# VISION-SJTU/UniDefense

Measured on AMD Instinct MI355X. Metric: images/sec fwd+bwd (256x256, EffNet-b4), higher is better.
Workload: dtype f32

## Files before the change

include/unidefense_hip.h:

```cpp
#ifndef UNIDEFENSE_HIP_H
#define UNIDEFENSE_HIP_H
#include <stdint.h>

#ifdef __cplusplus
extern "C" {
#endif

#define UD_EINVAL (-1000)

typedef void* ud_stream_t;

typedef struct {
    int N, Hin, Win, Cin, Hout, Wout, KH, KW, stride, pad_t, pad_l, transposed;
} ud_conv_geom;

typedef struct {
    const float* A; const float* B; float* C;
    int M, N, K;
    long lda, ldb, ldc;
    int a_mode, b_mode, out_mode, split_k;
    int batch; long strideA, strideB, strideC;
    ud_conv_geom g;
    double* stat_sum; double* stat_sumsq;
    int half_mask;
// ... 139 lines not shown
int ud_avgpool_fwd(const float* x, float* y, int N, int Ho, int Wo, int C, int k, ud_stream_t stream);
int ud_avgpool_bwd(const float* dy, float* dx, int N, int Ho, int Wo, int C, int k, ud_stream_t stream);
int ud_adaptive_avgpool_fwd(const float* x, float* y, int N, int H, int W, int Ho, int Wo, int C, ud_stream_t stream);
int ud_adaptive_avgpool_bwd(const float* dy, float* dx, int N, int H, int W, int Ho, int Wo, int C, ud_stream_t stream);
int ud_maxpool3s2_fwd(const float* x, float* y, unsigned char* arg, int N, int H, int W, int C,
                      ud_stream_t stream);
int ud_maxpool3s2_bwd(const float* dy, const unsigned char* arg, float* dx, int N, int H, int W, int C,
                      ud_stream_t stream);
int ud_add_act_fwd(const float* a, const float* b, int act, float* y, long total, ud_stream_t stream);
int ud_relu_bwd(const float* dy, const float* y, float* g, long total, ud_stream_t stream);
int ud_copy_cols(float* narrow, float* wide, long M, int Cn, int Cw, int off, int dir, ud_stream_t stream);

int ud_aw_triplet(const float* feat, int N, int D, int n_real, float* loss, float* dfeat, float* ws,
                  ud_stream_t stream);

typedef struct {
    const float* feat[3]; float* dfeat[3]; int D[3]; int nfeat;
    const float* cls; const long long* tgt; float* dcls; int N, C, R, F;
    const float* fm; float* dfm; int nfm; const float* sm; float* dsm; int nsm;
    const float* spatial; float* dspatial; const float* freq; float* dfreq;
    float w_cls, w_fm, w_sm, w_trip, w_rec, w_freq;
    float* vals;
    float* ws;
} ud_loss_tail;
int ud_loss_tail_ws_floats(int N, int n_real, int nfeat);
int ud_loss_tail_run(const ud_loss_tail* t, ud_stream_t stream);

int ud_conv_small_supported(int Cin, int Cout, int KH, int KW);
int ud_conv_small(const ud_conv_geom* g, const float* x, const float* wmat, float* y, int Cout, ud_stream_t stream);
int ud_conv_small_wgrad_supported(int Cin, int Ma, int KH, int KW);
long ud_conv_small_wgrad_ws_floats(int Cin, int Ma);
int ud_conv_small_wgrad(const ud_conv_geom* g, const float* a, const float* x, float* part, float* out, int Ma,
                        ud_stream_t stream);

int ud_stem_dgrad_supported(int Cin, int Cout, int KH, int KW, int stride);
int ud_stem_dgrad(const ud_conv_geom* g, const float* dy, const float* w, float* dx, int Cout, int accumulate,
                  ud_stream_t stream);
int ud_absdiff_bwd(const float* a, const float* b, const float* g, float* da, float* db, long total, ud_stream_t stream);
int ud_outer(const float* u, const float* v, float* out, long M, int D, ud_stream_t stream);

int ud_attack_step_linf(float* x_adv, const float* x0, const float* g, long total, float step, float eps, float lo, float hi,
                        ud_stream_t stream);
long ud_sample_sumsq_ws_bytes(int N, long per);
int ud_sample_sumsq(const float* a, const float* b, int N, long per, double* out, double* ws, long ws_bytes,
                    ud_stream_t stream);
int ud_attack_step_l2(float* x_adv, const float* g, const double* gss, int N, long per, float step, ud_stream_t stream);
int ud_attack_project_l2(float* x_adv, const float* x0, const double* dss, int N, long per, float eps, float lo, float hi,
                         ud_stream_t stream);

#define UD_APGD_MAX_CHECKPOINTS 16
#define UD_APGD_I_K 0
#define UD_APGD_I_CNT 1
#define UD_APGD_I_HALVED 2
#define UD_APGD_I_IMPROVED 3
#define UD_APGD_I_RESET 4
#define UD_APGD_F_PREV 0
#define UD_APGD_F_BEST 1
#define UD_APGD_F_CKPT 2
#define UD_APGD_F_ETA 3
#define UD_APGD_F_A 4
int ud_apgd_control(const float* f, int* ist, float* fst, float* history, int N, int steps, const int* ck_w,
                    const int* ck_thr, int n_ck, float eta0, float alpha, int closing, ud_stream_t stream);
int ud_apgd_update_linf(float* x, float* x_prev, float* x_best, float* g_best, const float* x0, const float* g, const int* ist,
                        const float* fst, int N, long per, float eps, float lo, float hi, ud_stream_t stream);
int ud_apgd_keep(float* dst, const float* src, const int* flag, int N, long per, ud_stream_t stream);
int ud_apgd_step_l2(float* x, float* z, float* x_best, float* g_best, double* gss_best, const float* g, const double* gss,
// ... 231 lines not shown
```

unidefense_amd/attack.py:

```python
import contextlib
import inspect
import math

import torch
import torch.nn.functional as F

from .infer import _MAX_RUNNERS, _check_model, _check_precision, _eval_nodes

DEFAULT_GRAD_SCALE = 1024.0

NORMS = ("linf", "l2")
OBJECTIVES = ("cross_entropy",)


def cross_entropy_sum(out, y):
    cls = out["cls_out"]
    if cls.shape[1] == 1:
        return F.binary_cross_entropy_with_logits(cls.squeeze(1), y.to(cls.dtype), reduction="sum")
    return F.cross_entropy(cls, y, reduction="sum")


def _objective(objective):
    if callable(objective):
        return objective
    if objective not in OBJECTIVES:
        raise ValueError(f"objective must be one of {OBJECTIVES} or a callable (out, y) -> scalar, got {objective!r}")
    return cross_entropy_sum


@contextlib.contextmanager
def frozen(model):
    flags = [(p, p.requires_grad) for p in model.parameters()]
    try:
# ... 63 lines not shown
    return objective if isinstance(objective, str) else getattr(objective, "__name__", repr(objective))


class _Runner:
    _what = "runner"
    _backward = True

    def _init_model(self, model, batch, size, precision, arguments):
        self.precision, self.half = precision, precision == "fp16"
        self.device = _check_model(self._what, model, precision, arguments)
        self.model, self.batch, self.size = model, int(batch), int(size)
        self.shape = (self.batch, 3, self.size, self.size)
        self.calls = 0
        self.graph = self.out = None

    def _init_loss(self, objective, grad_scale):
        self.grad_scale = resolve_grad_scale(self.precision, grad_scale)
        self.objective = _objective(objective)
        self.g = None

    def _check(self, x, y):
        if not isinstance(x, torch.Tensor) or not x.is_cuda or not isinstance(y, torch.Tensor) or not y.is_cuda:
            raise ValueError(f"{self._what} takes cuda tensors")
        if tuple(x.shape) != self.shape or x.dtype != torch.float32:
            raise ValueError(f"input {tuple(x.shape)} {x.dtype} differs from the runner's key {self.shape} torch.float32")
        if tuple(y.shape) != (self.batch,) or y.dtype != torch.int64:
            raise ValueError(f"labels {tuple(y.shape)} {y.dtype} differ from the runner's key ({self.batch},) torch.int64")
        if self.model.training:
            raise ValueError("the model is in training mode: call model.eval() before the runner")

    def _capture(self, *bodies):
        torch.cuda.synchronize(self.device)
        graphs = [torch.cuda.CUDAGraph() for _ in bodies]
        with frozen(self.model) if self._backward else contextlib.nullcontext():
            for g, body in zip(graphs, bodies):
                with torch.cuda.graph(g):
                    body()
        return graphs

    def _nodes(self):
        return _eval_nodes(self.model, half=True) if self.half else contextlib.nullcontext()

    def _grad(self, x, value):
        from . import kernels as K
        with self._nodes():
            out = self.model(x)
            f = value(out)
            total = f if f.dim() == 0 else f.sum()
            g, = torch.autograd.grad(total * self.grad_scale if self.half else total, x)
        if self.half:
            g = g.contiguous()
            K.axpby(g, 1.0 / self.grad_scale, out=g)
        return g, _detached(out), f

    def _each(self, out):
        f = self.objective(out, self.y)
        if not isinstance(f, torch.Tensor) or tuple(f.shape) != (self.batch,):
            raise ValueError(f"{self._what}'s objective must return a [{self.batch}] tensor, one value per sample, got "
                             f"{tuple(f.shape) if isinstance(f, torch.Tensor) else type(f).__name__}")
        return f

    def _draw(self, sample, generator):
        gdev = generator.device if generator is not None else self.device
        return sample(self.shape, generator=generator, device=gdev, dtype=torch.float32).to(self.device)

    def _box_start(self, x, generator):
        return (x + (self._draw(torch.rand, generator) * 2.0 - 1.0) * self.eps).clamp_(self.lo, self.hi)

    def _merge(self, restart, better):
        from . import kernels as K
# ... 635 lines not shown
```

unidefense_amd/kernels.py:

```python
import ctypes as C
import math
import os

import torch

from . import lib as _lib
from .config import cfg as CFG
from .devmem import Scratch, ZeroPool
from .lib import ConvGeom, GemmDesc, GemmP3Desc

_call = _lib.call

GEMM_PROFILE = None


def _stream():
    return C.c_void_p(torch.cuda.current_stream().cuda_stream)


def _p(t):
    if t is None:
        return None
    return C.c_void_p(t.data_ptr())

# ... 1046 lines not shown
def conv_geom(N, Hin, Win, Cin, Hout, Wout, KH, KW, stride, pad_t, pad_l, transposed=0):
    g = ConvGeom()
    g.N, g.Hin, g.Win, g.Cin, g.Hout, g.Wout = N, Hin, Win, Cin, Hout, Wout
    g.KH, g.KW, g.stride, g.pad_t, g.pad_l, g.transposed = KH, KW, stride, pad_t, pad_l, transposed
    return g


_CONV_SPLITK = True


_CONV_SMALL = True
_CONV_SMALL_MIN_M = 262144
_CONV_SMALL_OK = {}


def _conv_small_supported(Ci, Co, KH, KW):
    key = (Ci, Co, KH, KW)
    if key not in _CONV_SMALL_OK:
        _CONV_SMALL_OK[key] = _call("ud_conv_small_supported", Ci, Co, KH, KW) == 1
    return _CONV_SMALL_OK[key]


_CONV_SMALL_WS = Scratch(torch.float32)
_CONV_SMALL_WGRAD_OK = {}


def _conv_small_wgrad_supported(Ci, Ma, KH, KW):
    key = (Ci, Ma, KH, KW)
    if key not in _CONV_SMALL_WGRAD_OK:
        _CONV_SMALL_WGRAD_OK[key] = _call("ud_conv_small_wgrad_supported", Ci, Ma, KH, KW) == 1
    return _CONV_SMALL_WGRAD_OK[key]


def conv_gather_nt(x, wmat, g):
    _chk(x, wmat)
    M = g.N * g.Hout * g.Wout
    K = g.KH * g.KW * g.Cin
    Co = wmat.shape[0]
    assert wmat.shape[1] == K and x.numel() == g.N * g.Hin * g.Win * g.Cin
    if _CONV_SMALL and M >= _CONV_SMALL_MIN_M and _conv_small_supported(g.Cin, Co, g.KH, g.KW):
        out = empty((g.N, g.Hout, g.Wout, Co), x)
        _call("ud_conv_small", C.byref(g), _p(x), _p(wmat), _p(out), Co, _stream())
        return out
    split = _fwd_split(M, Co, K) if _CONV_SPLITK else 1
    if g.Cin % 4 == 0:
        gk = (g.Hin, g.Win, g.Cin, g.KH, g.KW, g.stride, g.transposed)
        tmp = []

        def scratch():
            if not tmp:
                tmp.append(empty((M, Co), x))
            return tmp[0]
        tuned = _tuned_plan(("conv",) + gk, M, Co, K,
                            lambda cfg, sp: _gemm(x, wmat, scratch(), M, Co, K, 0, K, Co, 2, 0, 2 if sp > 1 else 0, sp, geom=g, cfg=cfg),
                            lambda: _gemm(x, wmat, scratch(), M, Co, K, 0, K, Co, 2, 0, 2 if split > 1 else 0, split, geom=g))
        if tuned is not None:
            cfg, sp = tuned
            out = (split_out if sp > 1 else empty)((g.N, g.Hout, g.Wout, Co), x)
            _gemm(x, wmat, out, M, Co, K, 0, K, Co, 2, 0, 2 if sp > 1 else 0, sp, geom=g, cfg=cfg)
            return out
    if split > 1:
        out = split_out((g.N, g.Hout, g.Wout, Co), x)
        _gemm(x, wmat, out, M, Co, K, 0, K, Co, 2, 0, 2, split, geom=g)
        return out
    out = empty((g.N, g.Hout, g.Wout, Co), x)
    _gemm(x, wmat, out, M, Co, K, 0, K, Co, 2, 0, geom=g)
    return out


_STEM_DGRAD_OK = {}


# ... 266 lines not shown
def square_propose(x_try, x_best, x0, ist, side, dh, dw, dsign, eps, lo, hi, closing=False):
    _chk_same(x_try, x_best, x0)
    if x_try.dim() != 4 or x_try.shape[1] != 3 or x_try.shape[2] != x_try.shape[3]:
        raise ValueError(f"expected [N, 3, size, size] images, got {tuple(x_try.shape)}")
    N, size, steps = x_try.shape[0], x_try.shape[2], side.numel()
    _chk_state(ist, None, N, SQUARE_I, SQUARE_F)
    _chk_i32(side, (steps,), "side")
    _chk_i32(dh, (steps, N), "dh")
    _chk_i32(dw, (steps, N), "dw")
    _chk(dsign)
    if tuple(dsign.shape) != (steps, N, 3):
        raise ValueError(f"dsign must be [{steps}, {N}, 3], got {tuple(dsign.shape)}")
    _call("ud_square_propose", _p(x_try), _p(x_best), _p(x0), _p(ist), _p(side), _p(dh), _p(dw), _p(dsign), N, size, steps,
          float(eps), float(lo), float(hi), int(bool(closing)), _stream())
    return x_try


def square_control(f, ist, fst, history, decisions, steps, early_stop=True):
    _chk(f, history)
    N = f.numel()
    _chk_state(ist, fst, N, SQUARE_I, SQUARE_F)
    if tuple(history.shape) != (int(steps) + 1, N):
        raise ValueError(f"history must be [{int(steps) + 1}, {N}], got {tuple(history.shape)}")
    _chk_i32(decisions, (int(steps) + 1, N), "decisions")
    _call("ud_square_control", _p(f), _p(ist), _p(fst), _p(history), _p(decisions), N, int(steps), int(bool(early_stop)), _stream())


def conv_gather_wgrad(a, x, g):
    _chk(a, x)
    Kdim = g.N * g.Hout * g.Wout
    Ma = a.shape[-1]
    assert a.numel() == Kdim * Ma
    Ncols = g.KH * g.KW * g.Cin
    if _CONV_SMALL and Kdim >= _CONV_SMALL_MIN_M and _conv_small_wgrad_supported(g.Cin, Ma, g.KH, g.KW):
        ws = _CONV_SMALL_WS.get(a, _call("ud_conv_small_wgrad_ws_floats", g.Cin, Ma))
        out = empty((Ma, Ncols), a)
        _call("ud_conv_small_wgrad", C.byref(g), _p(a), _p(x), _p(ws), _p(out), Ma, _stream())
        return out
    split = _pick_split(_tiles(Ma, Ncols), Kdim)
    if g.Cin % 4 == 0 and Ma % 4 == 0:
        gk = (g.Hin, g.Win, g.Cin, g.KH, g.KW, g.stride, g.transposed)
        tmp = []

        def scratch():
            if not tmp:
                tmp.append(empty((Ma, Ncols), a))
            return tmp[0]
        tuned = _tuned_plan(("convw",) + gk, Ma, Ncols, Kdim,
                            lambda cfg, sp: _gemm(a, x, scratch(), Ma, Ncols, Kdim, Ma, 0, Ncols, 1, 2, 2 if sp > 1 else 0, sp, geom=g, cfg=cfg),
                            lambda: _gemm(a, x, scratch(), Ma, Ncols, Kdim, Ma, 0, Ncols, 1, 2, 2 if split > 1 else 0, split, geom=g))
        if tuned is not None:
            cfg, sp = tuned
            out = (split_out if sp > 1 else empty)((Ma, Ncols), a)
            return _gemm(a, x, out, Ma, Ncols, Kdim, Ma, 0, Ncols, 1, 2, 2 if sp > 1 else 0, sp, geom=g, cfg=cfg)
    if split > 1:
        out = split_out((Ma, Ncols), a)
        return _gemm(a, x, out, Ma, Ncols, Kdim, Ma, 0, Ncols, 1, 2, 2, split, geom=g)
    out = empty((Ma, Ncols), a)
    return _gemm(a, x, out, Ma, Ncols, Kdim, Ma, 0, Ncols, 1, 2, 0, 1, geom=g)


_REDUCE_WS = Scratch(torch.float64, 1 << 20)


def _ws64(ref, need):
    return _p(_REDUCE_WS.get(ref, need)) if need > 0 else None
# ... 1481 lines not shown
```

unidefense_amd/lib.py:

```python
import ctypes as C
import os

_HERE = os.path.dirname(os.path.abspath(__file__))
from .config import cfg as _cfg

LIB_PATH = _cfg.lib_path or os.path.join(_HERE, "libunidefense_hip.so")


class UDLibraryError(RuntimeError):
    pass


class ConvGeom(C.Structure):
    _fields_ = [(n, C.c_int) for n in ("N", "Hin", "Win", "Cin", "Hout", "Wout", "KH", "KW", "stride",
                                       "pad_t", "pad_l", "transposed")]


class GemmDesc(C.Structure):
    _fields_ = [("A", C.c_void_p), ("B", C.c_void_p), ("C", C.c_void_p),
                ("M", C.c_int), ("N", C.c_int), ("K", C.c_int),
                ("lda", C.c_long), ("ldb", C.c_long), ("ldc", C.c_long),
                ("a_mode", C.c_int), ("b_mode", C.c_int), ("out_mode", C.c_int), ("split_k", C.c_int),
                ("batch", C.c_int), ("strideA", C.c_long), ("strideB", C.c_long), ("strideC", C.c_long),
                ("g", ConvGeom), ("stat_sum", C.c_void_p), ("stat_sumsq", C.c_void_p), ("half_mask", C.c_int), ("tile_cfg", C.c_int), ("slice_stride", C.c_long)]
# ... 92 lines not shown
    "ud_gate_mix_fwd": [_P, _P, _P, _P, _L, _P],
    "ud_gate_mix_bwd": [_P, _P, _P, _P, _P, _P, _P, _P, _L, _P],
    "ud_residual_fwd": [_P, _P, _P, _F, _P, _L, _L, _P],
    "ud_axpby": [_P, _F, _P, _F, _P, _L, _I, _P],
    "ud_mask_scale": [_P, _P, _F, _P, _L, _P],
    "ud_absdiff": [_P, _P, _P, _L, _P],
    "ud_bcast_rows": [_P, _F, _P, _I, _I, _I, _P],
    "ud_pix_to_planes": [_P, _P, _I, _I, _I, _I, _P],
    "ud_planes_to_pix": [_P, _P, _P, _I, _I, _I, _I, _P],
    "ud_bilinear_fwd": [_P, _P, _I, _I, _I, _I, _I, _P],
    "ud_bilinear_bwd": [_P, _P, _I, _I, _I, _I, _I, _P],
    "ud_l1_chunks": [_L],
    "ud_l1_fwd": [_P, _P, _P, _P, _I, _L, _F, _P],
    "ud_l1_bwd": [_P, _P, _P, _F, _I, _P, _I, _L, _P],
    "ud_dynfilter_fwd": [_P, _P, _P, _P, _P, _P, _P, _P, _I, _I, _I, _I, _P],
    "ud_dynfilter_bwd": [_P, _P, _P, _P, _P, _P, _P, _P, _P, _I, _I, _I, _P],
    "ud_avgpool_fwd": [_P, _P, _I, _I, _I, _I, _I, _P],
    "ud_avgpool_bwd": [_P, _P, _I, _I, _I, _I, _I, _P],
    "ud_adaptive_avgpool_fwd": [_P, _P, _I, _I, _I, _I, _I, _I, _P],
    "ud_adaptive_avgpool_bwd": [_P, _P, _I, _I, _I, _I, _I, _I, _P],
    "ud_maxpool3s2_fwd": [_P, _P, _P, _I, _I, _I, _I, _P],
    "ud_maxpool3s2_bwd": [_P, _P, _P, _I, _I, _I, _I, _P],
    "ud_add_act_fwd": [_P, _P, _I, _P, _L, _P],
    "ud_relu_bwd": [_P, _P, _P, _L, _P],
    "ud_copy_cols": [_P, _P, _L, _I, _I, _I, _I, _P],
    "ud_aw_triplet": [_P, _I, _I, _I, _P, _P, _P, _P],
    "ud_loss_tail_ws_floats": [_I, _I, _I],
    "ud_loss_tail_run": [C.POINTER(LossTail), _P],
    "ud_conv_small_supported": [_I, _I, _I, _I],
    "ud_conv_small": [C.POINTER(ConvGeom), _P, _P, _P, _I, _P],
    "ud_conv_small_wgrad_supported": [_I, _I, _I, _I],
    "ud_conv_small_wgrad_ws_floats": [_I, _I],
    "ud_conv_small_wgrad": [C.POINTER(ConvGeom), _P, _P, _P, _P, _I, _P],
    "ud_stem_dgrad_supported": [_I, _I, _I, _I, _I],
    "ud_stem_dgrad": [C.POINTER(ConvGeom), _P, _P, _P, _I, _I, _P],
    "ud_attack_step_linf": [_P, _P, _P, _L, _F, _F, _F, _F, _P],
    "ud_sample_sumsq_ws_bytes": [_I, _L],
    "ud_sample_sumsq": [_P, _P, _I, _L, _P, _P, _L, _P],
    "ud_attack_step_l2": [_P, _P, _P, _I, _L, _F, _P],
    "ud_attack_project_l2": [_P, _P, _P, _I, _L, _F, _F, _F, _P],
    "ud_apgd_control": [_P, _P, _P, _P, _I, _I, C.POINTER(C.c_int), C.POINTER(C.c_int), _I, _F, _F, _I, _P],
    "ud_apgd_update_linf": [_P, _P, _P, _P, _P, _P, _P, _P, _I, _L, _F, _F, _F, _P],
    "ud_apgd_keep": [_P, _P, _P, _I, _L, _P],
    "ud_apgd_step_l2": [_P, _P, _P, _P, _P, _P, _P, _P, _P, _I, _L, _P],
    "ud_apgd_combine_l2": [_P, _P, _P, _P, _I, _L, _P],
    "ud_apgd_project_l2": [_P, _P, _P, _P, _I, _L, _F, _F, _F, _P],
    "ud_fmn_norms_ws_bytes": [_I, _L],
    "ud_fmn_norm_parts": [_P, _P, _P, _I, _L, _P, _L, _P],
    "ud_fmn_control": [_P, _P, _L, _P, _P, _P, _P, _P, _P, _P, _P, _I, _L, _I, _I, _I, _P],
    "ud_fmn_update": [_P, _P, _P, _P, _P, _P, _P, _I, _L, _I, _F, _F, _P],
    "ud_fmn_project_l2": [_P, _P, _P, _P, _I, _L, _F, _F, _P],
    "ud_square_propose": [_P, _P, _P, _P, _P, _P, _P, _P, _I, _I, _I, _F, _F, _F, _I, _P],
    "ud_square_control": [_P, _P, _P, _P, _P, _I, _I, _I, _P],
    "ud_absdiff_bwd": [_P, _P, _P, _P, _P, _L, _P],
    "ud_outer": [_P, _P, _P, _L, _I, _P],
    "ud_gather2d": [_P, _P, _P, _P, _L, _I, _I, _P],
    "ud_blur5_reflect": [_P, _P, _L, _I, _I, _F, _F, _F, _P],
    "ud_amp_mix": [_P, _P, _P, _P, _L, _I, _I, _I, _P],
    "ud_efdm_ws_bytes": [_I, _I],
    "ud_efdm": [_P, _P, _P, _P, _I, _I, _I, _P, _L, _P],
    "ud_coral_moments": [_P, _P, _I, _I, _I, _P],
    "ud_affine3": [_P, _P, _P, _I, _I, _P],
    "ud_fused_reduce_ws_doubles": [_I, _I, _I, _I, _I],
    "ud_colstats": [_P, _I, _I, _I, _P, _P, _P, _I, _P],
    "ud_colsum_bn": [_P, _BN, _I, _I, _I, _P, _P, _I, _P],
    "ud_coldot_bn": [_P, _P, _BN, _I, _I, _I, _P, _P, _I, _P],
# ... 41 lines not shown
    "ud_rfft2_ex": [_P, _P, _I, _I, _I, _F, _F, _BN, _P, _P, _I, _P, _P, _I, _P, _P],
    "ud_rfft2_ex_planes": [_P, _P, _L, _L, _P, _F, _P, _I, _I, _I, _F, _F, _BN, _P, _P, _I, _P, _P, _P, _P, _I, _P],
    "ud_irfft2_mix": [_P, _P, _I, _I, _I, _F, _F, _P, _P, _P, _P, _P, _I, _P],
    "ud_rfft2_two_pass": [_P, _P, _P, _I, _I, _I, _F, _F, _BN, _P, _P, _I, _P, _P, _I, _P, _P],
    "ud_irfft2_two_pass": [_P, _P, _P, _I, _I, _I, _F, _F, _P, _P, _P, _P, _P, _I, _P],
    "ud_fft2_two_pass_ws_floats": [_I, _I, _I],
    "ud_dwtile_ws_doubles": [_I, _I, _I, _I],
    "ud_dwtile": [_P, _BN, _P, _P] + [_I] * 10 + [_P, _I, _P, _P, _BN, _I, _P, _P, _P, _I, _I, _P],
    "ud_dwtile_wgrad_part_rows": [_I, _I, _I],
    "ud_dwtile_wgrad": [_P, _BN, _P, _P, _I, _P, _P, _L] + [_I] * 9 + [_I, _I, _P],
    "ud_dwtile_wgrad_finalize": [_P, _I, _I, _I, _P, _I, _P, _P],
    "ud_dwtile_wgrad_finalize_multi": [C.POINTER(WgradFold), _I, _P],
    "ud_rfft2_ex_plane_half": [_P, _P, _L, _P, _I, _I, _I, _F, _F, _BN, _P, _P, _I, _P, _P, _P, _P, _I, _P],
    "ud_irfft2_dwbwd": [_P, _I, _I, _I, _F, _F, _P, _P, _BN, _P, _I, _P, _I, _P, _P, _P, _P, _P, _I, _P],
    "ud_dwtile_dgrad_eval": [_P, _P, _P, _I, _P, _P, _BN, _P] + [_I] * 11 + [_P],
    "ud_dwtile_bwd": [_P, _P, _BN, _P, _P, _I, _P, _P, _P, _P, _L, _P, _P, _P] + [_I] * 8 + [_P],
    "ud_rfft2_planes_ws_floats": [_L, _I],
    "ud_rfft2_planes": [_P, _P, _P, _L, _I, _F, _P],
    "ud_rfft2_planes_adjoint": [_P, _P, _P, _L, _I, _F, _P],
    "ud_adamw_chunk_elems": [],
    "ud_adamw_multi": [_P, _P, _I, _P, _P, _I, C.c_double, C.c_double, C.c_double, _I, _I, _P, _P, _P, _P, _P],
    "ud_multi_add": [_P, _P, _P, _I, _P],
    "ud_gemm_get_path": [],
    "ud_sum_slices": [_P, _P, _I, _L, _L, _I, _P],
    "ud_xchg_bytes": [_I, _I, _I],
    "ud_xchg_create": [_I, _I, _I, _P, _P],
    "ud_xchg_open": [_P, _P],
    "ud_xchg_close": [_P],
    "ud_xchg_destroy": [_P],
    "ud_xchg_allreduce": [_P, _I, _P, _I, _I, _I, _I, _P, _P, _L, _P, _P],
}

_COUNT_FUNCS = {"ud_mb_eval_dw_ok", "ud_mb_eval_dw_tiles", "ud_mb_eval_dw_h_ok", "ud_mb_eval_dw_h_tiles", "ud_pj_fwd_fused_ok", "ud_pj_bwd_fused_ok", "ud_pj_bwd_fused_grid", "ud_pw_bwd_fused_ok", "ud_pw_bwd_fused_grid", "ud_loss_tail_ws_floats", "ud_dwtile_wgrad", "ud_dwtile_bwd", "ud_fft32_set_wave", "ud_fft2_two_pass_ws_floats", "ud_dwtile_ws_doubles", "ud_dwtile_wgrad_part_rows", "ud_reduce_ws_doubles", "ud_gemm_query_path", "ud_gemm_get_path", "ud_gemm_stats_slots", "ud_adamw_chunk_elems", "ud_rfft2_planes_ws_floats", "ud_fused_reduce_ws_doubles", "ud_dwconv_bwd_data_bn_ws_doubles", "ud_dwconv_bwd_weight_parts", "ud_sfmix_blocks", "ud_gate_mix_blocks",
                "ud_l1_chunks", "ud_efdm_ws_bytes", "ud_conv_small_supported", "ud_conv_small_wgrad_supported",
                "ud_conv_small_wgrad_ws_floats", "ud_xchg_bytes", "ud_stem_dgrad_supported", "ud_sample_sumsq_ws_bytes",
                "ud_coldot_bn_eval_ws_doubles", "ud_fmn_norms_ws_bytes"}
_LONG_FUNCS = {"ud_mb_eval_dw_tiles", "ud_mb_eval_dw_h_tiles", "ud_pj_bwd_fused_grid", "ud_pw_bwd_fused_grid", "ud_fft2_two_pass_ws_floats", "ud_dwtile_ws_doubles", "ud_dwtile_wgrad_part_rows", "ud_xchg_bytes", "ud_efdm_ws_bytes", "ud_rfft2_planes_ws_floats", "ud_conv_small_wgrad_ws_floats", "ud_fused_reduce_ws_doubles",
               "ud_dwconv_bwd_data_bn_ws_doubles", "ud_sample_sumsq_ws_bytes", "ud_coldot_bn_eval_ws_doubles",
               "ud_fmn_norms_ws_bytes"}

EXPORTED = tuple(_SIGNATURES)

_lib = None


def load():
    global _lib
    if _lib is not None:
        return _lib
    if not os.path.exists(LIB_PATH):
        raise UDLibraryError(
            f"{LIB_PATH} is missing: build it with `python -c 'import __graft_entry__ as g; g.build()'` "
            "or `make -C unidefense_amd/csrc`. unidefense_amd has no fallback path.")
    import torch
    if torch.cuda.is_available():
        torch.cuda.init()
    lib = C.CDLL(LIB_PATH)
    for name, argtypes in _SIGNATURES.items():
        fn = getattr(lib, name, None)
        if fn is None:
            raise UDLibraryError(f"{LIB_PATH} does not export {name}; rebuild it")
        fn.argtypes = argtypes
        fn.restype = C.c_long if name in _LONG_FUNCS else C.c_int
    _lib = lib
    return lib


def check(status: int, name: str):
    if status != 0:
        raise UDLibraryError(f"{name} failed with status {status}"
# ... 13 lines not shown
```

Baseline: 1326.

## Add MFMA split-fp16 implicit-GEMM 3x3 conv kernels for small-channel convs

Adds a HIP implicit-GEMM 3x3 conv kernel that stages input patches and weights in LDS as hi/lo fp16 pairs. It accumulates them with three 16x16x32 f16 MFMAs per product so fp32 accuracy is roughly preserved. Forward convs with small channel counts (20/40/80) at several strides are routed to it ahead of the existing small-conv path, and a weight-gradient variant is added but left disabled through an empty shape set. Garbage collection is also turned off during graph capture. The aim is to replace fp32 FMA or GEMM conv work with matrix-core throughput, at the cost of extra split arithmetic, per-stage rescaling and possible precision differences.

After: 1345 (median of 6 runs). 1.4% higher.

```diff
diff --git a/include/unidefense_hip.h b/include/unidefense_hip.h
--- a/include/unidefense_hip.h
+++ b/include/unidefense_hip.h
@@ -195,6 +195,14 @@
 long ud_conv_small_wgrad_ws_floats(int Cin, int Ma);
 int ud_conv_small_wgrad(const ud_conv_geom* g, const float* a, const float* x, float* part, float* out, int Ma,
                         ud_stream_t stream);
+
+int ud_conv_mfma_mode(const ud_conv_geom* g);
+int ud_conv_mfma_supported(int Cin, int Cout, int mode);
+int ud_conv_mfma(const ud_conv_geom* g, const float* x, const float* wmat, float* y, int Cout, ud_stream_t stream);
+int ud_conv_mfma_wgrad_supported(int Cin, int Ma, int mode);
+long ud_conv_mfma_wgrad_ws_floats(int Cin, int Ma);
+int ud_conv_mfma_wgrad(const ud_conv_geom* g, const float* a, const float* x, float* part, float* out, int Ma,
+                       ud_stream_t stream);
 
 int ud_stem_dgrad_supported(int Cin, int Cout, int KH, int KW, int stride);
 int ud_stem_dgrad(const ud_conv_geom* g, const float* dy, const float* w, float* dx, int Cout, int accumulate,
diff --git a/unidefense_amd/attack.py b/unidefense_amd/attack.py
--- a/unidefense_amd/attack.py
+++ b/unidefense_amd/attack.py
@@ -1,4 +1,5 @@
 import contextlib
+import gc
 import inspect
 import math
 
@@ -128,10 +129,16 @@
     def _capture(self, *bodies):
         torch.cuda.synchronize(self.device)
         graphs = [torch.cuda.CUDAGraph() for _ in bodies]
-        with frozen(self.model) if self._backward else contextlib.nullcontext():
-            for g, body in zip(graphs, bodies):
-                with torch.cuda.graph(g):
-                    body()
+        gc_was_on = gc.isenabled()
+        gc.disable()
+        try:
+            with frozen(self.model) if self._backward else contextlib.nullcontext():
+                for g, body in zip(graphs, bodies):
+                    with torch.cuda.graph(g):
+                        body()
+        finally:
+            if gc_was_on:
+                gc.enable()
         return graphs
 
     def _nodes(self):
diff --git a/unidefense_amd/csrc/conv_mfma.hip b/unidefense_amd/csrc/conv_mfma.hip
--- /dev/null
+++ b/unidefense_amd/csrc/conv_mfma.hip
@@ -0,0 +1,496 @@
+#include "pw_common.h"
+
+namespace {
+
+typedef _Float16 f16x2 __attribute__((ext_vector_type(2)));
+typedef _Float16 f16x8 __attribute__((ext_vector_type(8)));
+typedef uint32_t u32x2 __attribute__((ext_vector_type(2)));
+
+
+constexpr int odd_slots(int bytes) { return (bytes / 16) % 2 == 0 ? bytes + 16 : bytes; }
+constexpr int round_up(int v, int m) { return (v + m - 1) / m * m; }
+
+template <int CIN_, int COUT_, int MODE_, int TH_, int TW_, int CK_, int TS_, int NW_ = 4>
+struct Cfg {
+    static constexpr int CIN = CIN_, COUT = COUT_, MODE = MODE_, TH = TH_, TW = TW_, CK = CK_, TS = TS_, NW = NW_, NT = 64 * NW_;
+    static constexpr int CINP = round_up(CIN, 8), COUTP = round_up(COUT, 16), NTL = COUTP / 16;
+    static constexpr int PIX = TH * TW, MW = PIX / 16 / NW;
+    static constexpr int PH = MODE == 0 ? TH + 2 : MODE == 1 ? TH / 2 + 1 : 2 * TH + 1;
+    static constexpr int PW = MODE == 0 ? TW + 2 : MODE == 1 ? TW / 2 + 1 : 2 * TW + 1;
+    static constexpr int PROW = odd_slots(CINP * 2), PPLANE = PH * PW * PROW;
+    static constexpr int NCC = CIN / CK, NSTAGE = (9 / TS) * NCC;
+    static constexpr int CPT = round_up(CK, 8) / 8, NCH = TS * CPT;
+    static constexpr int KSTEPS = (NCH + 3) / 4, KSP = KSTEPS * 32;
+    static constexpr int WROW = odd_slots(KSP * 2), WPLANE = COUTP * WROW;
+    static constexpr int LDS = 2 * PPLANE + 2 * WPLANE;
+    static_assert(PIX % (16 * NW) == 0, "whole 16-pixel blocks for every wave");
+    static_assert(CIN % 4 == 0 && COUT % 4 == 0 && CK % 4 == 0, "16-byte runs");
+    static_assert(CIN % CK == 0 && (NCC == 1 || CK % 8 == 0) && 9 % TS == 0, "stages tile the reduction");
+    static_assert(MODE != 1 || (TS == 1 && TH % 2 == 0 && TW % 2 == 0 && (PIX / 4) % 16 == 0), "one parity per 16-pixel block");
+    static_assert(LDS + 64 <= 65536, "two workgroups per CU");
+};
+
+__device__ __forceinline__ float absmax4(float m, const f32x4& v) {
+    return fmaxf(fmaxf(m, fmaxf(fabsf(v[0]), fabsf(v[1]))), fmaxf(fabsf(v[2]), fabsf(v[3])));
+}
+__device__ __forceinline__ void store_split4h(char* dst, int plane, const f32x4& v, float s) {
+    uint32_t hi[2], lo[2];
+#pragma unroll
+    for (int h = 0; h < 2; ++h) {
+        const float a = v[2 * h] * s, b = v[2 * h + 1] * s;
+        const f16x2 p = {(_Float16)a, (_Float16)b};
+        const f16x2 q = {(_Float16)(a - (float)p[0]), (_Float16)(b - (float)p[1])};
+        hi[h] = __builtin_bit_cast(uint32_t, p);
+        lo[h] = __builtin_bit_cast(uint32_t, q);
+    }
+    *reinterpret_cast<u32x2*>(dst) = u32x2{hi[0], hi[1]};
+    *reinterpret_cast<u32x2*>(dst + plane) = u32x2{lo[0], lo[1]};
+}
+__device__ __forceinline__ float pow2f(int e) { return __uint_as_float((uint32_t)(127 + e) << 23); }
+
+template <class C>
+__global__ __launch_bounds__(C::NT) void conv_mfma(ud_conv_geom g, const float* __restrict__ x, const float* __restrict__ wmat,
+                                                float* __restrict__ y, int tiles_x, int tiles_y) {
+    constexpr int CIN = C::CIN, COUT = C::COUT, MODE = C::MODE, TH = C::TH, TW = C::TW, CK = C::CK, TS = C::TS;
+    constexpr int PW = C::PW, PROW = C::PROW, PPLANE = C::PPLANE, WROW = C::WROW, WPLANE = C::WPLANE;
+    constexpr int NT = C::NT, NW = C::NW;
+    constexpr int NTL = C::NTL, MW = C::MW, NCH = C::NCH, CPT = C::CPT, KSTEPS = C::KSTEPS, K = 9 * CIN;
+    __shared__ __attribute__((aligned(16))) char sm[C::LDS];
+    __shared__ float sred[2][4];
+    char* const patch = sm;
+    char* const ws = sm + 2 * PPLANE;
+    const int t = threadIdx.x, wave = t >> 6, lane = t & 63, pl = lane & 15, grp = lane >> 4;
+    int b = blockIdx.x;
+    const int tile_x = b % tiles_x;
+    b /= tiles_x;
+    const int tile_y = b % tiles_y, n = b / tiles_y;
+    const int oh0 = tile_y * TH, ow0 = tile_x * TW;
+    const int ih0 = MODE == 0 ? oh0 - 1 : MODE == 1 ? oh0 / 2 : 2 * oh0 - 1;
+    const int iw0 = MODE == 0 ? ow0 - 1 : MODE == 1 ? ow0 / 2 : 2 * ow0 - 1;
+
+    constexpr int WQ = C::KSP / 4, WITEMS = C::COUTP * WQ, NWI = (WITEMS + NT - 1) / NT;
+    f32x4 wr[NWI];
+    auto wload = [&](int stage) {
+        const int tap0 = (stage / C::NCC) * TS, c0 = (stage % C::NCC) * CK;
+#pragma unroll
+        for (int j = 0; j < NWI; ++j) {
+            const int i = t + j * NT;
+            const int co = i / WQ, c4 = i - co * WQ;
+            const int q = c4 >> 1, tl = q / CPT, cl = (q - tl * CPT) * 8 + (c4 & 1) * 4;
+            f32x4 v = {0.f, 0.f, 0.f, 0.f};
+            if (i < WITEMS && co < COUT && q < NCH && cl < CK)
+                v = *reinterpret_cast<const f32x4*>(wmat + (long)co * K + (tap0 + tl) * CIN + c0 + cl);
+            wr[j] = v;
+        }
+    };
+    wload(0);
+
+    float sx, inv_sx;
+    {
+        constexpr int CQ = C::CINP / 4, PITEMS = C::PH * PW * CQ, NPI = (PITEMS + NT - 1) / NT;
+        f32x4 pv[NPI];
+        float mx = 0.f;
+#pragma unroll
+        for (int j = 0; j < NPI; ++j) {
+            const int i = t + j * NT;
+            const int pix = i / CQ, c4 = i - pix * CQ;
+            const int py = pix / PW, px = pix - py * PW;
+            const int ih = ih0 + py, iw = iw0 + px;
+            f32x4 v = {0.f, 0.f, 0.f, 0.f};
+            if (i < PITEMS && c4 * 4 < CIN && ih >= 0 && ih < g.Hin && iw >= 0 && iw < g.Win)
+                v = *reinterpret_cast<const f32x4*>(x + (((long)n * g.Hin + ih) * g.Win + iw) * CIN + c4 * 4);
+            pv[j] = v;
+            mx = absmax4(mx, v);
+        }
+        mx = ud_wave_max(mx);
+        if (lane == 0) sred[1][wave] = mx;
+        __syncthreads();
+        mx = sred[1][0];
+#pragma unroll
+        for (int w = 1; w < NW; ++w) mx = fmaxf(mx, sred[1][w]);
+        ud_h2_scale(__float_as_uint(mx), sx, inv_sx);
+#pragma unroll
+        for (int j = 0; j < NPI; ++j) {
+            const int i = t + j * NT;
+            const int pix = i / CQ, c4 = i - pix * CQ;
+            if (i < PITEMS) store_split4h(patch + pix * PROW + c4 * 8, PPLANE, pv[j], sx);
+        }
+    }
+
+    int ty[MW], tx[MW];
+#pragma unroll
+    for (int mi = 0; mi < MW; ++mi) {
+        const int p = (wave + NW * mi) * 16 + pl;
+        if (MODE == 1) {
+            constexpr int PC = C::PIX / 4, HW = TW / 2;
+            const int cls = p / PC, r = p - cls * PC;
+            ty[mi] = 2 * (r / HW) + (cls >> 1);
+            tx[mi] = 2 * (r % HW) + (cls & 1);
+        } else {
+            ty[mi] = p / TW;
+            tx[mi] = p % TW;
+        }
+    }
+
+    f32x4 acc[MW][NTL];
+#pragma unroll
+    for (int mi = 0; mi < MW; ++mi)
+#pragma unroll
+        for (int nt = 0; nt < NTL; ++nt) acc[mi][nt] = f32x4{0.f, 0.f, 0.f, 0.f};
+
+    int swe = 0, smin = 0;
+    bool have = false;
+#pragma unroll 1
+    for (int stage = 0; stage < C::NSTAGE; ++stage) {
+        const int tap0 = (stage / C::NCC) * TS, c0 = (stage % C::NCC) * CK;
+        float mw = 0.f;
+#pragma unroll
+        for (int j = 0; j < NWI; ++j) mw = absmax4(mw, wr[j]);
+        mw = ud_wave_max(mw);
+        if (lane == 0) sred[stage & 1][wave] = mw;
+        __syncthreads();
+        mw = sred[stage & 1][0];
+#pragma unroll
+        for (int w = 1; w < NW; ++w) mw = fmaxf(mw, sred[stage & 1][w]);
+        int ratio_e = 0;
+        {
+            const uint32_t bits = __float_as_uint(mw);
+            const int ef = (int)(bits >> 23) & 0xff;
+            if (ef != 0) {
+                int want = 14 - (ef - 127);
+                want = want < -100 ? -100 : want > 100 ? 100 : want;
+                if (!have) {
+                    swe = smin = want;
+                    have = true;
+                } else {
+                    const int top = ef - 127 + swe;
+                    if (top > 14 || top < 4) {
+                        const int ne = want < smin + 80 ? want : smin + 80;
+                        ratio_e = ne - swe;
+                        swe = ne;
+                        smin = ne < smin ? ne : smin;
+                    }
+                }
+            }
+        }
+        const float sw = pow2f(swe);
+#pragma unroll
+        for (int j = 0; j < NWI; ++j) {
+            const int i = t + j * NT;
+            const int co = i / WQ, c4 = i - co * WQ;
+            if (i < WITEMS) store_split4h(ws + co * WROW + c4 * 8, WPLANE, wr[j], sw);
+        }
+        if (stage + 1 < C::NSTAGE) wload(stage + 1);
+        __syncthreads();
+        if (ratio_e != 0) {
+            const float ratio = pow2f(ratio_e < -126 ? -126 : ratio_e);
+#pragma unroll
+            for (int mi = 0; mi < MW; ++mi)
+#pragma unroll
+                for (int nt = 0; nt < NTL; ++nt) acc[mi][nt] *= ratio;
+        }
+        bool act[MW];
+        bool any = false;
+#pragma unroll
+        for (int mi = 0; mi < MW; ++mi) {
+            act[mi] = true;
+            if (MODE == 1) {
+                const int cls = (wave + NW * mi) / (C::PIX / 64);
+                const int kh = tap0 / 3, kw = tap0 - 3 * kh;
+                act[mi] = ((kh & 1) != (cls >> 1)) && ((kw & 1) != (cls & 1));
+            }
+            any = any || act[mi];
+        }
+        if (!any) continue;
+#pragma unroll
+        for (int ks = 0; ks < KSTEPS; ++ks) {
+            const int q = ks * 4 + grp;
+            f16x8 wf[NTL][2];
+#pragma unroll
+            for (int nt = 0; nt < NTL; ++nt) {
+                const char* s = ws + (nt * 16 + pl) * WROW + q * 16;
+                wf[nt][0] = *reinterpret_cast<const f16x8*>(s);
+                wf[nt][1] = *reinterpret_cast<const f16x8*>(s + WPLANE);
+            }
+            const int qc = q < NCH ? q : NCH - 1;
+            const int tl = qc / CPT, c8 = qc - tl * CPT;
+            const int tap = tap0 + tl, kh = tap / 3, kw = tap - 3 * kh;
+            const int coff = (c0 + c8 * 8) * 2;
+#pragma unroll
+            for (int mi = 0; mi < MW; ++mi) {
+                if (!act[mi]) continue;
+                int py, px;
+                if (MODE == 0) {
+                    py = ty[mi] + kh;
+                    px = tx[mi] + kw;
+                } else if (MODE == 1) {
+                    py = (ty[mi] + 1 - kh) >> 1;
+                    px = (tx[mi] + 1 - kw) >> 1;
+                } else {
+                    py = 2 * ty[mi] + kh;
+                    px = 2 * tx[mi] + kw;
+                }
+                const char* s = patch + (py * PW + px) * PROW + coff;
+                const f16x8 xh = *reinterpret_cast<const f16x8*>(s);
+                const f16x8 xl = *reinterpret_cast<const f16x8*>(s + PPLANE);
+#pragma unroll
+                for (int nt = 0; nt < NTL; ++nt) {
+                    f32x4 c = acc[mi][nt];
+                    c = __builtin_amdgcn_mfma_f32_16x16x32_f16(wf[nt][1], xh, c, 0, 0, 0);
+                    c = __builtin_amdgcn_mfma_f32_16x16x32_f16(wf[nt][0], xl, c, 0, 0, 0);
+                    c = __builtin_amdgcn_mfma_f32_16x16x32_f16(wf[nt][0], xh, c, 0, 0, 0);
+                    acc[mi][nt] = c;
+                }
+            }
+        }
+    }
+
+    const float inv_sw = pow2f(-swe);
+#pragma unroll
+    for (int mi = 0; mi < MW; ++mi) {
+        const int oh = oh0 + ty[mi], ow = ow0 + tx[mi];
+        if (oh >= g.Hout || ow >= g.Wout) continue;
+        float* dst = y + (((long)n * g.Hout + oh) * g.Wout + ow) * COUT;
+#pragma unroll
+        for (int nt = 0; nt < NTL; ++nt) {
+            const int co = nt * 16 + grp * 4;
+            if (co < COUT) *reinterpret_cast<f32x4*>(dst + co) = acc[mi][nt] * inv_sw * inv_sx;
+        }
+    }
+}
+
+template <class C>
+int launch(const ud_conv_geom& g, const float* x, const float* wmat, float* y, hipStream_t s) {
+    const int tiles_x = ud_cdiv(g.Wout, C::TW), tiles_y = ud_cdiv(g.Hout, C::TH);
+    const long blocks = (long)g.N * tiles_x * tiles_y;
+    if (blocks > 0x7fffffffL) return UD_EINVAL;
+    hipLaunchKernelGGL((conv_mfma<C>), dim3((unsigned)blocks), dim3(C::NT), 0, s, g, x, wmat, y, tiles_x, tiles_y);
+    UD_LAUNCH_CHECK();
+    return 0;
+}
+
+
+template <int CIN_, int MA_, int MODE_, int CC_>
+struct WCfg {
+    static constexpr int CIN = CIN_, MA = MA_, MODE = MODE_, CC = CC_, S = MODE == 0 ? 1 : 2;
+    static constexpr int PH = 3 * S + 3, PWP = 7 * S + 3;
+    static constexpr int MAP = round_up(MA, 16), MT = MAP / 16, NY = CIN / CC;
+    static constexpr int NC = 9 * CC, NTILES = round_up(NC, 16) / 16, NTW = (NTILES + 3) / 4;
+    static constexpr int AROW = 80, APLANE = MAP * AROW;
+    static constexpr int XPLANE = 3 * CC * PH * 16;
+    static constexpr int LDS = 3 * APLANE + 3 * XPLANE;
+    static_assert(MODE == 0 || MODE == 2, "gathers of a plain conv: stride 1 or 2, pad 1");
+    static_assert(CIN % CC == 0 && CC % 4 == 0 && MA % 4 == 0, "16-byte runs");
+    static_assert(LDS <= 65536, "two workgroups per CU");
+};
+
+__device__ __forceinline__ void store_split4t(char* dst, int plane, int stride, const f32x4& v) {
+    uint32_t p[2][3];
+    pw::split2(v[0], v[1], p[0][0], p[0][1], p[0][2]);
+    pw::split2(v[2], v[3], p[1][0], p[1][1], p[1][2]);
+#pragma unroll
+    for (int c = 0; c < 4; ++c)
+#pragma unroll
+        for (int k = 0; k < 3; ++k) {
+            const uint32_t w = p[c >> 1][k];
+            *reinterpret_cast<uint16_t*>(dst + c * stride + k * plane) = (uint16_t)((c & 1) ? (w >> 16) : (w & 0xffffu));
+        }
+}
+
+template <class C>
+__global__ __launch_bounds__(256) void conv_mfma_wgrad(ud_conv_geom g, const float* __restrict__ a, const float* __restrict__ x,
+                                                       float* __restrict__ part, int tiles_x, int tiles_y, int ntiles) {
+    constexpr int CIN = C::CIN, MA = C::MA, CC = C::CC, S = C::S, PH = C::PH, PWP = C::PWP, MT = C::MT, NTW = C::NTW;
+    constexpr int AROW = C::AROW, APLANE = C::APLANE, XPLANE = C::XPLANE, NC = C::NC, K = 9 * CIN;
+    __shared__ __attribute__((aligned(16))) char sm[C::LDS];
+    char* const at = sm;
+    char* const xs = sm + 3 * APLANE;
+    const int t = threadIdx.x, wave = t >> 6, lane = t & 63, pl = lane & 15, grp = lane >> 4;
+    const int c0 = blockIdx.y * CC;
+    f32x4 acc[MT][NTW];
+#pragma unroll
+    for (int mt = 0; mt < MT; ++mt)
+#pragma unroll
+        for (int j = 0; j < NTW; ++j) acc[mt][j] = f32x4{0.f, 0.f, 0.f, 0.f};
+    int xoff[NTW];
+#pragma unroll
+    for (int j = 0; j < NTW; ++j) {
+        int c = (wave + 4 * j) * 16 + pl;
+        c = c < NC ? c : NC - 1;
+        const int tap = c / CC, ci = c - tap * CC, kh = tap / 3, kw = tap - 3 * kh;
+        xoff[j] = ((kw * CC + ci) * PH + S * grp + kh) * 16;
+    }
+    for (int tile = blockIdx.x; tile < ntiles; tile += gridDim.x) {
+        int b = tile;
+        const int tile_x = b % tiles_x;
+        b /= tiles_x;
+        const int tile_y = b % tiles_y, n = b / tiles_y;
+        const int oh0 = tile_y * 4, ow0 = tile_x * 8, ih0 = S * oh0 - 1, iw0 = S * ow0 - 1;
+        __syncthreads();
+        {
+            constexpr int Q = C::MAP / 4, ITEMS = 32 * Q;
+            for (int i = t; i < ITEMS; i += 256) {
+                const int p = i / Q, c4 = i - p * Q;
+                const int oh = oh0 + (p >> 3), ow = ow0 + (p & 7);
+                f32x4 v = {0.f, 0.f, 0.f, 0.f};
+                if (c4 * 4 < MA && oh < g.Hout && ow < g.Wout)
+                    v = *reinterpret_cast<const f32x4*>(a + (((long)n * g.Hout + oh) * g.Wout + ow) * MA + c4 * 4);
+                store_split4t(at + c4 * 4 * AROW + p * 2, APLANE, AROW, v);
+            }
+        }
+        {
+            constexpr int Q = CC / 4, ITEMS = PH * PWP * Q;
+            for (int i = t; i < ITEMS; i += 256) {
+                const int pix = i / Q, c4 = i - pix * Q;
+                const int py = pix / PWP, px = pix - py * PWP;
+                const int ih = ih0 + py, iw = iw0 + px;
+                f32x4 v = {0.f, 0.f, 0.f, 0.f};
+                if (ih >= 0 && ih < g.Hin && iw >= 0 && iw < g.Win)
+                    v = *reinterpret_cast<const f32x4*>(x + (((long)n * g.Hin + ih) * g.Win + iw) * CIN + c0 + c4 * 4);
+#pragma unroll
+                for (int kw = 0; kw < 3; ++kw) {
+                    const int d = px - kw;
+                    if (d >= 0 && d % S == 0 && d / S < 8)
+                        store_split4t(xs + ((kw * CC + c4 * 4) * PH + py) * 16 + (d / S) * 2, XPLANE, PH * 16, v);
+                }
+            }
+        }
+        __syncthreads();
+        pw::Frag3 af[MT];
+#pragma unroll
+        for (int mt = 0; mt < MT; ++mt) {
+            const char* sp = at + (mt * 16 + pl) * AROW + grp * 16;
+#pragma unroll
+            for (int k = 0; k < 3; ++k) af[mt].p[k] = *reinterpret_cast<const pw::bf16x8*>(sp + k * APLANE);
+        }
+#pragma unroll
+        for (int j = 0; j < NTW; ++j) {
+            if ((wave + 4 * j) * 16 >= NC) continue;
+            pw::Frag3 bf;
+#pragma unroll
+            for (int k = 0; k < 3; ++k) bf.p[k] = *reinterpret_cast<const pw::bf16x8*>(xs + xoff[j] + k * XPLANE);
+#pragma unroll
+            for (int mt = 0; mt < MT; ++mt) acc[mt][j] = pw::mma6(af[mt], bf, acc[mt][j]);
+        }
+    }
+    float* dst = part + (long)blockIdx.x * MA * K;
+#pragma unroll
+    for (int j = 0; j < NTW; ++j) {
+        const int c = (wave + 4 * j) * 16 + pl;
+        if (c >= NC) continue;
+        const int tap = c / CC, ci = c - tap * CC;
+#pragma unroll
+        for (int mt = 0; mt < MT; ++mt)
+#pragma unroll
+            for (int r = 0; r < 4; ++r) {
+                const int ma = mt * 16 + grp * 4 + r;
+                if (ma < MA) dst[(long)ma * K + tap * CIN + c0 + ci] = acc[mt][j][r];
+            }
+    }
+}
+
+int wgrad_parts(long ntiles, int Cin, int Ma, int ny) {
+    long cap = 6L * 1024 * 1024 / ((long)Ma * 9 * Cin);
+    if (cap > 512 / ny) cap = 512 / ny;
+    long p = ntiles / 4;
+    if (p > cap) p = cap;
+    return p < 1 ? 1 : (int)p;
+}
+
+template <class C>
+int launch_wgrad(const ud_conv_geom& g, const float* a, const float* x, float* part, float* out, hipStream_t s) {
+    const int tiles_x = ud_cdiv(g.Wout, 8), tiles_y = ud_cdiv(g.Hout, 4);
+    const long ntiles = (long)g.N * tiles_x * tiles_y;
+    if (ntiles > 0x7fffffffL) return UD_EINVAL;
+    const int parts = wgrad_parts(ntiles, C::CIN, C::MA, C::NY);
+    hipLaunchKernelGGL((conv_mfma_wgrad<C>), dim3((unsigned)parts, (unsigned)C::NY), dim3(256), 0, s, g, a, x, part, tiles_x, tiles_y,
+                       (int)ntiles);
+    UD_LAUNCH_CHECK();
+    return pw::fold_launch(part, parts, C::MA * 9 * C::CIN, out, nullptr, nullptr, 0, nullptr, nullptr, s);
+}
+
+int mode_of(const ud_conv_geom& g) {
+    if (g.KH != 3 || g.KW != 3 || g.pad_t != 1 || g.pad_l != 1) return -1;
+    if (!g.transposed && g.stride == 1 && g.Hout == g.Hin && g.Wout == g.Win) return 0;
+    if (g.transposed && g.stride == 2 && g.Hout == 2 * g.Hin && g.Wout == 2 * g.Win) return 1;
+    if (!g.transposed && g.stride == 2 && g.Hin == 2 * g.Hout && g.Win == 2 * g.Wout) return 2;
+    return -1;
+}
+
+}
+
+#define UD_CONV_MFMA_CASES(X)                                                                   \
+    X(20, 20, 0, 16, 16, 20, 9, 4)                                                  \
+    X(40, 20, 0, 8, 16, 40, 3, 4)                                                   \
+    X(40, 40, 0, 8, 16, 40, 3, 4)                                                   \
+    X(20, 40, 0, 8, 16, 20, 9, 4)                                                   \
+    X(80, 40, 0, 8, 8, 80, 1, 4)                                                    \
+    X(80, 80, 0, 8, 8, 40, 1, 4)                                                    \
+    X(40, 80, 0, 8, 8, 40, 3, 4)                                                    \
+    X(160, 80, 0, 4, 8, 40, 1, 2)    \
+    X(80, 160, 0, 4, 8, 16, 1, 2)                                    \
+    X(20, 20, 1, 16, 16, 20, 1, 4)                                                  \
+    X(40, 40, 1, 16, 16, 40, 1, 4)                                                  \
+    X(80, 80, 1, 8, 16, 80, 1, 4)                                                   \
+    X(20, 20, 2, 8, 8, 20, 9, 4)                                                    \
+    X(40, 40, 2, 8, 8, 40, 1, 4)                                                    \
+    X(80, 80, 2, 4, 4, 40, 1, 1)
+
+extern "C" {
+
+int ud_conv_mfma_mode(const ud_conv_geom* g) { return g ? mode_of(*g) : -1; }
+
+int ud_conv_mfma_supported(int Cin, int Cout, int mode) {
+#define X(ci, co, m, th, tw, ck, ts, nw) \
+    if (Cin == ci && Cout == co && mode == m) return 1;
+    UD_CONV_MFMA_CASES(X)
+#undef X
+    return 0;
+}
+
+int ud_conv_mfma(const ud_conv_geom* g, const float* x, const float* wmat, float* y, int Cout, ud_stream_t stream) {
+    if (!g || !x || !wmat || !y) return UD_EINVAL;
+    const int mode = mode_of(*g);
+    if (mode < 0 || !ud_conv_mfma_supported(g->Cin, Cout, mode)) return UD_EINVAL;
+    if ((((uintptr_t)x | (uintptr_t)wmat | (uintptr_t)y) & 15) != 0) return UD_EINVAL;
+    if (g->N < 1 || g->Hout < 1 || g->Wout < 1) return 0;
+    hipStream_t s = (hipStream_t)stream;
+#define X(ci, co, m, th, tw, ck, ts, nw) \
+    if (g->Cin == ci && Cout == co && mode == m) return launch<Cfg<ci, co, m, th, tw, ck, ts, nw>>(*g, x, wmat, y, s);
+    UD_CONV_MFMA_CASES(X)
+#undef X
+    return UD_EINVAL;
+}
+
+#define UD_CONV_MFMA_WGRAD_CASES(X) \
+    X(160, 80, 0, 40) X(80, 80, 0, 40) X(80, 40, 0, 40) X(40, 40, 0, 40) X(40, 20, 0, 40) X(20, 20, 0, 20) \
+    X(80, 80, 2, 20) X(40, 40, 2, 20) X(20, 20, 2, 20)
+
+int ud_conv_mfma_wgrad_supported(int Cin, int Ma, int mode) {
+#define X(ci, ma, m, cc) \
+    if (Cin == ci && Ma == ma && mode == m) return 1;
+    UD_CONV_MFMA_WGRAD_CASES(X)
+#undef X
+    return 0;
+}
+
+long ud_conv_mfma_wgrad_ws_floats(int Cin, int Ma) {
+    if (Cin < 1 || Ma < 1) return UD_EINVAL;
+    return (long)wgrad_parts(1L << 40, Cin, Ma, 1) * Ma * 9 * Cin;
+}
+
+int ud_conv_mfma_wgrad(const ud_conv_geom* g, const float* a, const float* x, float* part, float* out, int Ma, ud_stream_t stream) {
+    if (!g || !a || !x || !part || !out) return UD_EINVAL;
+    const int mode = mode_of(*g);
+    if (mode < 0 || !ud_conv_mfma_wgrad_supported(g->Cin, Ma, mode)) return UD_EINVAL;
+    if ((((uintptr_t)a | (uintptr_t)x) & 15) != 0) return UD_EINVAL;
+    if (g->N < 1 || g->Hout < 1 || g->Wout < 1) return UD_EINVAL;
+    hipStream_t s = (hipStream_t)stream;
+#define X(ci, ma, m, cc) \
+    if (g->Cin == ci && Ma == ma && mode == m) return launch_wgrad<WCfg<ci, ma, m, cc>>(*g, a, x, part, out, s);
+    UD_CONV_MFMA_WGRAD_CASES(X)
+#undef X
+    return UD_EINVAL;
+}
+
+}
diff --git a/unidefense_amd/kernels.py b/unidefense_amd/kernels.py
--- a/unidefense_amd/kernels.py
+++ b/unidefense_amd/kernels.py
@@ -1102,12 +1102,54 @@
     return _CONV_SMALL_WGRAD_OK[key]
 
 
+_CONV_MFMA = True
+_CONV_MFMA_MIN_M = 16384
+_CONV_MFMA_SHAPES = frozenset({(20, 20, 0), (40, 20, 0), (40, 40, 0), (20, 40, 0), (80, 40, 0), (80, 80, 0), (40, 80, 0),
+                               (20, 20, 1), (40, 40, 1), (80, 80, 1), (20, 20, 2)})
+_CONV_MFMA_OK = {}
+
+
+def _conv_mfma_mode(g):
+    return int(_lib.load().ud_conv_mfma_mode(C.byref(g)))
+
+
+def _conv_mfma_takes(g, Co, M, *tensors):
+    if not _CONV_MFMA or M < _CONV_MFMA_MIN_M:
+        return False
+    key = (g.Cin, Co, _conv_mfma_mode(g))
+    if key[2] < 0 or (_CONV_MFMA_SHAPES is not None and key not in _CONV_MFMA_SHAPES):
+        return False
+    if key not in _CONV_MFMA_OK:
+        _CONV_MFMA_OK[key] = _call("ud_conv_mfma_supported", *key) == 1
+    return _CONV_MFMA_OK[key] and all(t.dtype == torch.float32 and t.data_ptr() % 16 == 0 for t in tensors)
+
+
+_CONV_MFMA_WGRAD_SHAPES = frozenset()
+_CONV_MFMA_WGRAD_OK = {}
+_CONV_MFMA_WS = Scratch(torch.float32)
+
+
+def _conv_mfma_wgrad_takes(g, Ma, M, *tensors):
+    if not _CONV_MFMA or M < _CONV_MFMA_MIN_M:
+        return False
+    key = (g.Cin, Ma, _conv_mfma_mode(g))
+    if key[2] not in (0, 2) or (_CONV_MFMA_WGRAD_SHAPES is not None and key not in _CONV_MFMA_WGRAD_SHAPES):
+        return False
+    if key not in _CONV_MFMA_WGRAD_OK:
+        _CONV_MFMA_WGRAD_OK[key] = _call("ud_conv_mfma_wgrad_supported", *key) == 1
+    return _CONV_MFMA_WGRAD_OK[key] and all(t.dtype == torch.float32 and t.data_ptr() % 16 == 0 for t in tensors)
+
+
 def conv_gather_nt(x, wmat, g):
     _chk(x, wmat)
     M = g.N * g.Hout * g.Wout
     K = g.KH * g.KW * g.Cin
     Co = wmat.shape[0]
     assert wmat.shape[1] == K and x.numel() == g.N * g.Hin * g.Win * g.Cin
+    if _conv_mfma_takes(g, Co, M, x, wmat):
+        out = empty((g.N, g.Hout, g.Wout, Co), x)
+        _call("ud_conv_mfma", C.byref(g), _p(x), _p(wmat), _p(out), Co, _stream())
+        return out
     if _CONV_SMALL and M >= _CONV_SMALL_MIN_M and _conv_small_supported(g.Cin, Co, g.KH, g.KW):
         out = empty((g.N, g.Hout, g.Wout, Co), x)
         _call("ud_conv_small", C.byref(g), _p(x), _p(wmat), _p(out), Co, _stream())
@@ -1440,6 +1482,11 @@
     Ma = a.shape[-1]
     assert a.numel() == Kdim * Ma
     Ncols = g.KH * g.KW * g.Cin
+    if _conv_mfma_wgrad_takes(g, Ma, Kdim, a, x):
+        ws = _CONV_MFMA_WS.get(a, _call("ud_conv_mfma_wgrad_ws_floats", g.Cin, Ma))
+        out = empty((Ma, Ncols), a)
+        _call("ud_conv_mfma_wgrad", C.byref(g), _p(a), _p(x), _p(ws), _p(out), Ma, _stream())
+        return out
     if _CONV_SMALL and Kdim >= _CONV_SMALL_MIN_M and _conv_small_wgrad_supported(g.Cin, Ma, g.KH, g.KW):
         ws = _CONV_SMALL_WS.get(a, _call("ud_conv_small_wgrad_ws_floats", g.Cin, Ma))
         out = empty((Ma, Ncols), a)
diff --git a/unidefense_amd/lib.py b/unidefense_amd/lib.py
--- a/unidefense_amd/lib.py
+++ b/unidefense_amd/lib.py
@@ -148,6 +148,12 @@
     "ud_conv_small_wgrad_supported": [_I, _I, _I, _I],
     "ud_conv_small_wgrad_ws_floats": [_I, _I],
     "ud_conv_small_wgrad": [C.POINTER(ConvGeom), _P, _P, _P, _P, _I, _P],
+    "ud_conv_mfma_mode": [C.POINTER(ConvGeom)],
+    "ud_conv_mfma_supported": [_I, _I, _I],
+    "ud_conv_mfma": [C.POINTER(ConvGeom), _P, _P, _P, _I, _P],
+    "ud_conv_mfma_wgrad_supported": [_I, _I, _I],
+    "ud_conv_mfma_wgrad_ws_floats": [_I, _I],
+    "ud_conv_mfma_wgrad": [C.POINTER(ConvGeom), _P, _P, _P, _P, _I, _P],
     "ud_stem_dgrad_supported": [_I, _I, _I, _I, _I],
     "ud_stem_dgrad": [C.POINTER(ConvGeom), _P, _P, _P, _I, _I, _P],
     "ud_attack_step_linf": [_P, _P, _P, _L, _F, _F, _F, _F, _P],
@@ -255,10 +261,10 @@
 }
 
 _COUNT_FUNCS = {"ud_mb_eval_dw_ok", "ud_mb_eval_dw_tiles", "ud_mb_eval_dw_h_ok", "ud_mb_eval_dw_h_tiles", "ud_pj_fwd_fused_ok", "ud_pj_bwd_fused_ok", "ud_pj_bwd_fused_grid", "ud_pw_bwd_fused_ok", "ud_pw_bwd_fused_grid", "ud_loss_tail_ws_floats", "ud_dwtile_wgrad", "ud_dwtile_bwd", "ud_fft32_set_wave", "ud_fft2_two_pass_ws_floats", "ud_dwtile_ws_doubles", "ud_dwtile_wgrad_part_rows", "ud_reduce_ws_doubles", "ud_gemm_query_path", "ud_gemm_get_path", "ud_gemm_stats_slots", "ud_adamw_chunk_elems", "ud_rfft2_planes_ws_floats", "ud_fused_reduce_ws_doubles", "ud_dwconv_bwd_data_bn_ws_doubles", "ud_dwconv_bwd_weight_parts", "ud_sfmix_blocks", "ud_gate_mix_blocks",
-                "ud_l1_chunks", "ud_efdm_ws_bytes", "ud_conv_small_supported", "ud_conv_small_wgrad_supported",
+                "ud_l1_chunks", "ud_efdm_ws_bytes", "ud_conv_small_supported", "ud_conv_small_wgrad_supported", "ud_conv_mfma_supported", "ud_conv_mfma_wgrad_supported", "ud_conv_mfma_wgrad_ws_floats",
                 "ud_conv_small_wgrad_ws_floats", "ud_xchg_bytes", "ud_stem_dgrad_supported", "ud_sample_sumsq_ws_bytes",
                 "ud_coldot_bn_eval_ws_doubles", "ud_fmn_norms_ws_bytes"}
-_LONG_FUNCS = {"ud_mb_eval_dw_tiles", "ud_mb_eval_dw_h_tiles", "ud_pj_bwd_fused_grid", "ud_pw_bwd_fused_grid", "ud_fft2_two_pass_ws_floats", "ud_dwtile_ws_doubles", "ud_dwtile_wgrad_part_rows", "ud_xchg_bytes", "ud_efdm_ws_bytes", "ud_rfft2_planes_ws_floats", "ud_conv_small_wgrad_ws_floats", "ud_fused_reduce_ws_doubles",
+_LONG_FUNCS = {"ud_mb_eval_dw_tiles", "ud_mb_eval_dw_h_tiles", "ud_pj_bwd_fused_grid", "ud_pw_bwd_fused_grid", "ud_fft2_two_pass_ws_floats", "ud_dwtile_ws_doubles", "ud_dwtile_wgrad_part_rows", "ud_xchg_bytes", "ud_efdm_ws_bytes", "ud_rfft2_planes_ws_floats", "ud_conv_small_wgrad_ws_floats", "ud_conv_mfma_wgrad_ws_floats", "ud_fused_reduce_ws_doubles",
                "ud_dwconv_bwd_data_bn_ws_doubles", "ud_sample_sumsq_ws_bytes", "ud_coldot_bn_eval_ws_doubles",
                "ud_fmn_norms_ws_bytes"}
 
```
